# Advanced-Vision-and-Learning-Lab/sparse-view-3dgs-pack

Measured on AMD Instinct MI355X. Metric: train-step views/s (fwd+bwd) @1M Gaussians 1080p, higher is better.
Workload: dtype f32

## Files before the change

### sparse-view-3dgs-pack_amd/csrc/gs_blend.h

```cpp
#pragma once
#include <hip/hip_runtime.h>

#define GS_LOG2E 1.4426950408889634f

__device__ __forceinline__ float4 blend_stage_conic(float4 conic_o) {
  return make_float4(-0.5f * GS_LOG2E * conic_o.x, -GS_LOG2E * conic_o.y, -0.5f * GS_LOG2E * conic_o.z, conic_o.w);
}
__device__ __forceinline__ float blend_power2(float4 q, float dx, float dy) {
  const float t = fmaf(q.y, dy, q.x * dx);
  return fmaf(q.z * dy, dy, t * dx);
}
__device__ __forceinline__ float blend_exp2(float p2) { return __builtin_amdgcn_exp2f(p2); }
```

### sparse-view-3dgs-pack_amd/csrc/gs_render_bwd_wave.hip

```cpp
#include "gs_blend.h"
#include "gs_common.h"

template <int CTRL, int ROW_MASK, bool BOUND>
__device__ __forceinline__ float dppw(float v) {
  return __builtin_bit_cast(
      float, __builtin_amdgcn_update_dpp(0, __builtin_bit_cast(int, v), CTRL, ROW_MASK, 0xf, BOUND));
}
typedef unsigned uint2v __attribute__((ext_vector_type(2)));
__device__ __forceinline__ float swap32_add(float a, float b) {
  const uint2v r = __builtin_amdgcn_permlane32_swap(__builtin_bit_cast(unsigned, a), __builtin_bit_cast(unsigned, b), false, false);
  const unsigned x = r[0], y = r[1];
  return __uint_as_float(x) + __uint_as_float(y);
}
__device__ __forceinline__ float swap16_add(float a, float b) {
  const uint2v r = __builtin_amdgcn_permlane16_swap(__builtin_bit_cast(unsigned, a), __builtin_bit_cast(unsigned, b), false, false);
  const unsigned x = r[0], y = r[1];
  return __uint_as_float(x) + __uint_as_float(y);
}
__device__ __forceinline__ float row_total_in_lane15(float v) {
  v += dppw<0x111, 0xf, true>(v);
  v += dppw<0x112, 0xf, true>(v);
  v += dppw<0x114, 0xf, true>(v);
  v += dppw<0x118, 0xf, true>(v);
  return v;
}
__device__ __forceinline__ float row_total_in_lane0(float v) {
  v += dppw<0x101, 0xf, true>(v);
  v += dppw<0x102, 0xf, true>(v);
  v += dppw<0x104, 0xf, true>(v);
  v += dppw<0x108, 0xf, true>(v);
  return v;
}

#define WB 64

template <bool HAS_INVDEPTH, bool HAS_EXTRA, bool FSGS>
__global__ void __launch_bounds__(64, (HAS_INVDEPTH || HAS_EXTRA) ? 3 : 4) render_bwd_wave_kernel(
    const uint2* __restrict__ ranges, const uint32_t* __restrict__ point_list, int W, int H, int grid_x,
    const Splat* __restrict__ splat, const float* __restrict__ bg, const float* __restrict__ final_Ts,
    const uint32_t* __restrict__ n_contrib, const uint32_t* __restrict__ tile_work,
    const uint32_t* __restrict__ tile_order, const float* __restrict__ dL_dpixels,
    const float* __restrict__ dL_invdepths, const float* __restrict__ dL_dextra, gs_row_t* __restrict__ grad_rows) {
  __shared__ float4 s_a[WB];
  __shared__ float4 s_c[WB];
  __shared__ float4 s_k[WB];
  __shared__ uint32_t s_id[WB];

  const uint32_t tile_u = tile_order[blockIdx.x];
  if (tile_u == 0xFFFFFFFFu) return;
  const int tile = (int)tile_u;
  const uint32_t lmax = tile_work[tile];
  if (lmax == 0) return;
  const int tile_x = tile % grid_x, tile_y = tile / grid_x;
  const int lane = threadIdx.x;
  const uint2 range = ranges[tile];
  const int n = (int)(range.y - range.x);
  if (n == 0) return;

  const int px0 = tile_x * TILE_X + (lane & 7), py0 = tile_y * TILE_Y + (lane >> 3);
  const float pixfx0 = (float)px0, pixfy0 = (float)py0;
  const size_t HW = (size_t)H * W;

  float T[4], Tbg[4], dLp0[4], dLp1[4], dLp2[4], dLinv[4], dLpX[4];
  float A[4], kd_prev[4], last_alpha[4];
  uint32_t lastc[4];
#pragma unroll
  for (int s = 0; s < 4; s++) {
    const int px = px0 + (s & 1) * 8, py = py0 + (s >> 1) * 8;
    const bool inside = px < W && py < H;
    const int pix_id = W * py + px;
    T[s] = inside ? final_Ts[pix_id] : 0.f;
    lastc[s] = inside ? n_contrib[pix_id] : 0u;
    dLp0[s] = inside ? dL_dpixels[pix_id] : 0.f;
    dLp1[s] = inside ? dL_dpixels[HW + pix_id] : 0.f;
    dLp2[s] = inside ? dL_dpixels[2 * HW + pix_id] : 0.f;
    dLinv[s] = (HAS_INVDEPTH && inside) ? dL_invdepths[pix_id] : 0.f;
    dLpX[s] = (HAS_EXTRA && inside) ? dL_dextra[pix_id] : 0.f;
    float b = 0;
    if (HAS_EXTRA && !FSGS) b += bg[0] * dLpX[s];
    b += bg[0] * dLp0[s];
    b += bg[1] * dLp1[s];
    b += bg[2] * dLp2[s];
    Tbg[s] = T[s] * b;
    A[s] = kd_prev[s] = last_alpha[s] = 0.f;
  }
  const int rq = lane >> 4, lr = lane & 15;
  const float rowscale0 = rq == 0 ? (0.5f * W) / GS_LOG2E : (rq == 1 ? (0.5f * H) / GS_LOG2E : -0.5f);
  const float rowscale1 = rq == 0 ? -0.5f : 1.0f;
  const bool live2 = rq == 0 || (HAS_EXTRA && !FSGS && rq == 1) || (HAS_INVDEPTH && rq == 2);
  const int lane_slot = lr == 15 ? rq : (lr == 0 ? 4 + rq : (rq == 0 ? GR_CB : (rq == 1 ? GR_EXTRA : (rq == 2 ? GR_ID : GR_N))));
  const float lane_scale = lr == 15 ? rowscale0 : (lr == 0 ? rowscale1 : 1.0f);
  const bool lane_adds = lr == 15 || lr == 0 || (lr == 7 && live2);
  const int q0 = n - (int)lmax;
  const int rounds = (n + WB - 1) / WB;

  float4 ra, rc, rk;
  uint32_t rid = 0;
  ra = rc = rk = make_float4(0.f, 0.f, 0.f, 0.f);
  {
    const int q = (q0 / WB) * WB + lane;
    if (q < n) {
      rid = point_list[range.y - q - 1];
      const float4* rec = reinterpret_cast<const float4*>(&splat[rid]);
      ra = rec[0]; rc = rec[1]; rk = rec[2];
    }
  }
  for (int i = q0 / WB; i < rounds; i++) {
    __syncthreads();
    s_id[lane] = rid;
    s_a[lane] = make_float4(ra.x, ra.y, FSGS ? ra.z : ra.w, 0.f);
    s_c[lane] = blend_stage_conic(rc);
    s_k[lane] = FSGS ? make_float4(rk.x, rk.y, rk.z, 1.0f) : rk;
    __syncthreads();
    {
      const int q = (i + 1) * WB + lane;
      if (q < n) {
        rid = point_list[range.y - q - 1];
        const float4* rec = reinterpret_cast<const float4*>(&splat[rid]);
        ra = rec[0]; rc = rec[1]; rk = rec[2];
      }
    }
    const int cnt = min(WB, n - i * WB);
    const int jbeg = max(0, q0 - i * WB);
    for (int j = jbeg; j < cnt; j++) {
      const uint32_t contributor = (uint32_t)(n - 1 - (i * WB + j));
      const float4 a = s_a[j];
      const float4 co = s_c[j];
      float G[4], alpha[4];
      bool valid[4];
      unsigned long long vmask[4];
#pragma unroll
      for (int s = 0; s < 4; s++) {
        const float dx = a.x - (pixfx0 + (float)((s & 1) * 8));
        const float dy = a.y - (pixfy0 + (float)((s >> 1) * 8));
        const float p2 = blend_power2(co, dx, dy);
        G[s] = blend_exp2(p2);
        alpha[s] = fminf(0.99f, co.w * G[s]);
        const bool c0 = contributor < lastc[s], c1 = p2 <= 0.0f, c2 = alpha[s] >= 1.0f / 255.0f;
        valid[s] = c0 && c1 && c2;
        vmask[s] = __ballot(c0) & __ballot(c1) & __ballot(c2);
      }
      if ((vmask[0] | vmask[1] | vmask[2] | vmask[3]) == 0ull) continue;

      float v_mx = 0.f, v_my = 0.f, v_cxx = 0.f, v_cxy = 0.f, v_cyy = 0.f, v_op = 0.f;
      float v_c0 = 0.f, v_c1 = 0.f, v_c2 = 0.f, v_id = 0.f, v_x = 0.f;
      const float4 k = s_k[j];
      const float q2a = co.x + co.x, q2c = co.z + co.z;
#pragma unroll
      for (int s = 0; s < 4; s++) {
        if (valid[s]) {
          const float dx = a.x - (pixfx0 + (float)((s & 1) * 8));
          const float dy = a.y - (pixfy0 + (float)((s >> 1) * 8));
          const float om = 1.f - alpha[s];
          float rinv = __builtin_amdgcn_rcpf(om);
          rinv = fmaf(rinv, fmaf(-om, rinv, 1.0f), rinv);
          T[s] = T[s] * rinv;
          const float w = alpha[s] * T[s];
          A[s] = fmaf(last_alpha[s], kd_prev[s] - A[s], A[s]);
          float kd = k.x * dLp0[s];
          kd = fmaf(k.y, dLp1[s], kd);
          kd = fmaf(k.z, dLp2[s], kd);
          v_c0 = fmaf(w, dLp0[s], v_c0);
          v_c1 = fmaf(w, dLp1[s], v_c1);
          v_c2 = fmaf(w, dLp2[s], v_c2);
          if (HAS_INVDEPTH) {
            kd = fmaf(a.z, dLinv[s], kd);
            v_id = fmaf(w, dLinv[s], v_id);
          }
          if (HAS_EXTRA) {
            kd = fmaf(k.w, dLpX[s], kd);
            v_x = fmaf(w, dLpX[s], v_x);
          }
          kd_prev[s] = kd;
          const float dL_dalpha = fmaf(kd - A[s], T[s], -Tbg[s] * rinv);
          last_alpha[s] = alpha[s];
          v_op = fmaf(G[s], dL_dalpha, v_op);
          const float h = co.w * G[s] * dL_dalpha;
          const float hx = h * dx, hy = h * dy;
          v_cxx = fmaf(hx, dx, v_cxx);
          v_cxy = fmaf(hx, dy, v_cxy);
          v_cyy = fmaf(hy, dy, v_cyy);
          v_mx = fmaf(q2a, hx, fmaf(co.y, hy, v_mx));
          v_my = fmaf(q2c, hy, fmaf(co.y, hx, v_my));
        }
      }
      const float s0 = swap32_add(v_mx, v_cxx), s1 = swap32_add(v_my, v_cxy);
      const float s2 = swap32_add(v_cyy, v_c0), s3 = swap32_add(v_op, v_c1);
      const float s4 = swap32_add(v_c2, v_id);
      const float t0 = row_total_in_lane15(swap16_add(s0, s1));
      const float t1 = row_total_in_lane0(swap16_add(s2, s3));
      const float s5 = HAS_EXTRA ? swap32_add(v_x, 0.f) : 0.f;
      const float t2 = row_total_in_lane15(swap16_add(s4, s5));
      const float t2m = dppw<0x128, 0xf, true>(t2);
      const float tot = (lr == 15 ? t0 : (lr == 0 ? t1 : t2m)) * lane_scale;
      if (lane_adds) atomicAdd(grad_rows + (size_t)s_id[j] * GR_STRIDE + lane_slot, (double)tot);
    }
  }
}

__global__ void __launch_bounds__(64) blend_stats_kernel(const uint2* __restrict__ ranges, const uint32_t* __restrict__ point_list,
                                                         int W, int H, int grid_x, const Splat* __restrict__ splat,
                                                         const uint32_t* __restrict__ n_contrib,
                                                         const uint32_t* __restrict__ tile_work,
                                                         unsigned long long* __restrict__ out) {
  const int tile = blockIdx.x;
  const uint32_t lmax = tile_work[tile];
  if (lmax == 0) return;
  const int tile_x = tile % grid_x, tile_y = tile / grid_x;
  const int lane = threadIdx.x;
  const uint2 range = ranges[tile];
  const int n = (int)(range.y - range.x);
  if (n == 0) return;
  const int px0 = tile_x * TILE_X + (lane & 7), py0 = tile_y * TILE_Y + (lane >> 3);
  uint32_t lastc[4];
  for (int s = 0; s < 4; s++) {
    const int px = px0 + (s & 1) * 8, py = py0 + (s >> 1) * 8;
    lastc[s] = (px < W && py < H) ? n_contrib[W * py + px] : 0u;
  }
  unsigned long long c_vis = 0, c_any = 0, c_quad = 0, c_pix = 0;
  for (int q = n - (int)lmax; q < n; q++) {
    const uint32_t contributor = (uint32_t)(n - 1 - q);
    const uint32_t id = point_list[range.y - q - 1];
    const float4* rec = reinterpret_cast<const float4*>(&splat[id]);
    const float4 ra = rec[0];
    const float4 co = blend_stage_conic(rec[1]);
    c_vis++;
    int quads = 0;
    for (int s = 0; s < 4; s++) {
      const float dx = ra.x - (float)(px0 + (s & 1) * 8), dy = ra.y - (float)(py0 + (s >> 1) * 8);
      const float p2 = blend_power2(co, dx, dy);
      const float alpha = fminf(0.99f, co.w * blend_exp2(p2));
      const bool valid = contributor < lastc[s] && p2 <= 0.0f && alpha >= 1.0f / 255.0f;
      const unsigned long long m = __ballot(valid);
      if (m) quads++;
      c_pix += (unsigned long long)__popcll(m);
    }
    c_quad += quads;
    c_any += quads ? 1 : 0;
  }
  if (lane == 0) {
    atomicAdd(&out[0], c_vis);
    atomicAdd(&out[1], c_any);
    atomicAdd(&out[2], c_quad);
    atomicAdd(&out[3], c_pix);
    atomicAdd(&out[4], 1ull);
    atomicAdd(&out[5], (unsigned long long)n);
  }
}
int launch_blend_stats(const uint2* ranges, const uint32_t* point_list, int W, int H, int grid_x, int grid_y, const Splat* splat,
                       const uint32_t* n_contrib, const uint32_t* tile_work, unsigned long long* out, hipStream_t s) {
  hipLaunchKernelGGL(blend_stats_kernel, dim3(grid_x * grid_y), dim3(64), 0, s, ranges, point_list, W, H, grid_x, splat, n_contrib,
                     tile_work, out);
  return 0;
}

__global__ void __launch_bounds__(GS_BLOCK) zero_rows_kernel(float4* __restrict__ p, size_t P,
                                                             const uint32_t* __restrict__ tiles_touched) {
  const size_t i = (size_t)blockIdx.x * GS_BLOCK + threadIdx.x;
  if (i >= P || (tiles_touched && tiles_touched[i] == 0)) return;
  float4* w = p + i * (GR_ROW_BYTES / 16);
  w[0] = w[1] = w[2] = w[3] = w[4] = w[5] = make_float4(0.f, 0.f, 0.f, 0.f);
}
int launch_zero_rows(gs_row_t* rows, size_t P, const uint32_t* tiles_touched, hipStream_t s) {
  static_assert(GR_ROW_BYTES == 128, "eight float4 per row, six in use");
  if (P) hipLaunchKernelGGL(zero_rows_kernel, dim3((unsigned)((P + GS_BLOCK - 1) / GS_BLOCK)), dim3(GS_BLOCK), 0, s,
                            reinterpret_cast<float4*>(rows), P, tiles_touched);
  return 0;
}

int launch_render_bwd_wave(const uint2* ranges, const uint32_t* point_list, int W, int H, int grid_x, int grid_y,
                           const Splat* splat, const float* bg, const float* final_T, const uint32_t* n_contrib,
                           const uint32_t* tile_work, const uint32_t* tile_order, const float* dL_dpix,
                           const float* dL_dinvdepth, const float* dL_dextra, gs_row_t* grad_rows, int fsgs, hipStream_t s) {
#define GS_BWD_WAVE(ID, EX, FS)                                                                                           \
  hipLaunchKernelGGL((render_bwd_wave_kernel<ID, EX, FS>), dim3(((grid_x * grid_y + 7) / 8) * 8), dim3(64), 0, s, ranges, point_list, W, H, \
                     grid_x, splat, bg, final_T, n_contrib, tile_work, tile_order, dL_dpix, dL_dinvdepth, dL_dextra, grad_rows)
  if (fsgs) GS_BWD_WAVE(true, true, true);
  else if (dL_dinvdepth && dL_dextra) GS_BWD_WAVE(true, true, false);
  else if (dL_dinvdepth) GS_BWD_WAVE(true, false, false);
  else if (dL_dextra) GS_BWD_WAVE(false, true, false);
  else GS_BWD_WAVE(false, false, false);
#undef GS_BWD_WAVE
  return 0;
}
```

Baseline: 1172.

## Prefetch splat records into LDS via async global_load_lds in backward blend

Replaces the register-staged prefetch and the two __syncthreads per round in the wave-sized backward kernel with direct global-to-LDS DMA loads (global_load_lds). Point IDs are fetched three rounds ahead into a 4-deep ring and splat records one round ahead into a double buffer, with hand-managed vmcnt waits that count the outstanding atomics. The aim is to hide the gather latency of point_list and splat records and remove barrier and VGPR staging overhead. The cost is fragile inline asm and manual waitcnt accounting. Stale-tail clamped loads and the in-place conic transform also depend on single-wave ordering.

```diff
diff --git a/sparse-view-3dgs-pack_amd/csrc/gs_blend.h b/sparse-view-3dgs-pack_amd/csrc/gs_blend.h
--- a/sparse-view-3dgs-pack_amd/csrc/gs_blend.h
+++ b/sparse-view-3dgs-pack_amd/csrc/gs_blend.h
@@ -11,3 +11,23 @@
   return fmaf(q.z * dy, dy, t * dx);
 }
 __device__ __forceinline__ float blend_exp2(float p2) { return __builtin_amdgcn_exp2f(p2); }
+
+__device__ __forceinline__ uint32_t lds_addr(const void* p) {
+  return (uint32_t)(uintptr_t)(const __attribute__((address_space(3))) void*)p;
+}
+__device__ __forceinline__ void lds_dma_dword(const void* g, uint32_t lds) {
+  asm volatile("s_nop 0\n\tglobal_load_lds_dword %0, off" ::"v"(g), "{m0}"(lds) : "memory");
+}
+__device__ __forceinline__ void lds_dma_dwordx4(const void* g, uint32_t lds) {
+  asm volatile("s_nop 0\n\tglobal_load_lds_dwordx4 %0, off" ::"v"(g), "{m0}"(lds) : "memory");
+}
+template <int FLOOR>
+__device__ __forceinline__ void blend_vm_wait(int younger) {
+  static_assert(FLOOR == 0 || FLOOR == 1, "rungs");
+  if (younger >= 63) asm volatile("s_waitcnt vmcnt(63)" ::: "memory");
+  else if (younger >= 32) asm volatile("s_waitcnt vmcnt(32)" ::: "memory");
+  else if (younger >= 16) asm volatile("s_waitcnt vmcnt(16)" ::: "memory");
+  else if (younger >= 8) asm volatile("s_waitcnt vmcnt(8)" ::: "memory");
+  else if (FLOOR == 1) asm volatile("s_waitcnt vmcnt(1)" ::: "memory");
+  else asm volatile("s_waitcnt vmcnt(0)" ::: "memory");
+}
diff --git a/sparse-view-3dgs-pack_amd/csrc/gs_render_bwd_wave.hip b/sparse-view-3dgs-pack_amd/csrc/gs_render_bwd_wave.hip
--- a/sparse-view-3dgs-pack_amd/csrc/gs_render_bwd_wave.hip
+++ b/sparse-view-3dgs-pack_amd/csrc/gs_render_bwd_wave.hip
@@ -41,10 +41,8 @@
     const uint32_t* __restrict__ n_contrib, const uint32_t* __restrict__ tile_work,
     const uint32_t* __restrict__ tile_order, const float* __restrict__ dL_dpixels,
     const float* __restrict__ dL_invdepths, const float* __restrict__ dL_dextra, gs_row_t* __restrict__ grad_rows) {
-  __shared__ float4 s_a[WB];
-  __shared__ float4 s_c[WB];
-  __shared__ float4 s_k[WB];
-  __shared__ uint32_t s_id[WB];
+  __shared__ float4 s_rec[2][3][WB];
+  __shared__ uint32_t s_ids[4][WB];
 
   const uint32_t tile_u = tile_order[blockIdx.x];
   if (tile_u == 0xFFFFFFFFu) return;
@@ -94,32 +92,39 @@
   const int q0 = n - (int)lmax;
   const int rounds = (n + WB - 1) / WB;
 
-  float4 ra, rc, rk;
-  uint32_t rid = 0;
-  ra = rc = rk = make_float4(0.f, 0.f, 0.f, 0.f);
-  {
-    const int q = (q0 / WB) * WB + lane;
-    if (q < n) {
-      rid = point_list[range.y - q - 1];
-      const float4* rec = reinterpret_cast<const float4*>(&splat[rid]);
-      ra = rec[0]; rc = rec[1]; rk = rec[2];
+  const uint32_t ids_lds = __builtin_amdgcn_readfirstlane(lds_addr(&s_ids[0][0]));
+  const uint32_t rec_lds = __builtin_amdgcn_readfirstlane(lds_addr(&s_rec[0][0][0]));
+  auto issue_ids = [&](int b) {
+    const int q = min(b * WB + lane, n - 1);
+    lds_dma_dword(point_list + (range.y - q - 1), ids_lds + (uint32_t)((b & 3) * WB * 4));
+  };
+  auto issue_records = [&](int b) {
+    const float4* rec = reinterpret_cast<const float4*>(splat + s_ids[b & 3][lane]);
+    const uint32_t dst = rec_lds + (uint32_t)((b & 1) * 3 * WB * 16);
+    lds_dma_dwordx4(rec, dst);
+    lds_dma_dwordx4(rec + 1, dst + WB * 16);
+    lds_dma_dwordx4(rec + 2, dst + 2 * WB * 16);
+  };
+  const int i0 = q0 / WB;
+  issue_ids(i0);
+  issue_ids(i0 + 1);
+  blend_vm_wait<1>(1);
+  issue_records(i0);
+  issue_ids(i0 + 2);
+  int atomics = 0;
+  for (int i = i0; i < rounds; i++) {
+    blend_vm_wait<1>(1 + atomics);
+    atomics = 0;
+    {
+      float4* c = &s_rec[i & 1][1][lane];
+      *c = blend_stage_conic(*c);
     }
-  }
-  for (int i = q0 / WB; i < rounds; i++) {
-    __syncthreads();
-    s_id[lane] = rid;
-    s_a[lane] = make_float4(ra.x, ra.y, FSGS ? ra.z : ra.w, 0.f);
-    s_c[lane] = blend_stage_conic(rc);
-    s_k[lane] = FSGS ? make_float4(rk.x, rk.y, rk.z, 1.0f) : rk;
-    __syncthreads();
-    {
-      const int q = (i + 1) * WB + lane;
-      if (q < n) {
-        rid = point_list[range.y - q - 1];
-        const float4* rec = reinterpret_cast<const float4*>(&splat[rid]);
-        ra = rec[0]; rc = rec[1]; rk = rec[2];
-      }
-    }
+    issue_records(i + 1);
+    issue_ids(i + 3);
+    const float4* s_a = s_rec[i & 1][0];
+    const float4* s_c = s_rec[i & 1][1];
+    const float4* s_k = s_rec[i & 1][2];
+    const uint32_t* s_id = s_ids[i & 3];
     const int cnt = min(WB, n - i * WB);
     const int jbeg = max(0, q0 - i * WB);
     for (int j = jbeg; j < cnt; j++) {
@@ -164,11 +169,11 @@
           v_c1 = fmaf(w, dLp1[s], v_c1);
           v_c2 = fmaf(w, dLp2[s], v_c2);
           if (HAS_INVDEPTH) {
-            kd = fmaf(a.z, dLinv[s], kd);
+            kd = fmaf(FSGS ? a.z : a.w, dLinv[s], kd);
             v_id = fmaf(w, dLinv[s], v_id);
           }
           if (HAS_EXTRA) {
-            kd = fmaf(k.w, dLpX[s], kd);
+            kd = fmaf(FSGS ? 1.0f : k.w, dLpX[s], kd);
             v_x = fmaf(w, dLpX[s], v_x);
           }
           kd_prev[s] = kd;
@@ -194,8 +199,10 @@
       const float t2m = dppw<0x128, 0xf, true>(t2);
       const float tot = (lr == 15 ? t0 : (lr == 0 ? t1 : t2m)) * lane_scale;
       if (lane_adds) atomicAdd(grad_rows + (size_t)s_id[j] * GR_STRIDE + lane_slot, (double)tot);
+      atomics++;
     }
   }
+  blend_vm_wait<0>(atomics);
 }
 
 __global__ void __launch_bounds__(64) blend_stats_kernel(const uint2* __restrict__ ranges, const uint32_t* __restrict__ point_list,
```

Result: no change. 1172 (median of 4 runs) (+0.0%).
